# Maxwell-Zhao/RoboSimGS

Hardware: AMD Instinct MI355X
Metric: frames/sec + ms/frame (fwd, fwd+bwd) at 1M Gaussians 1920x1080 (higher is better)
Workload: dtype f32

## Files before the change

### robosimgs_amd/csrc/binning.hip

```cpp
#include "mgs_common.h"
#include "tile_rect.h"
#include "tile_order.h"

namespace mgs {
namespace {

constexpr int kBlock = 128;

__device__ __forceinline__ uint32_t wave_sum(uint32_t v) {
#pragma unroll
  for (int d = 32; d >= 1; d >>= 1) v += __shfl_xor(v, d);
  return v;
}

constexpr int kSum = 64;
__global__ __launch_bounds__(kBlock) void tile_count_kernel(
    int n, const float* __restrict__ means2d, const int32_t* __restrict__ radii,
    const int32_t* __restrict__ radii_y, const float* __restrict__ conics, const float* __restrict__ opacities,
    float tile_size, int tile_w, int tile_h, uint2* __restrict__ ginfo, uint32_t* __restrict__ sums) {
  int g = blockIdx.x * kBlock + threadIdx.x;
  int radius = g < n ? radii[g] : 0;
  uint2 info = make_uint2(kEmptyTileRect, 0u);
  if (radius > 0) {
    float2 m = reinterpret_cast<const float2*>(means2d)[g];
    TileRect r = tile_rect(m.x, m.y, radius, radii_y ? radii_y[g] : radius, tile_size, tile_w, tile_h);
    if (conics)
      r = tighten_rect(r, m.x, m.y, conics[3 * (size_t)g], conics[3 * (size_t)g + 1],
                       conics[3 * (size_t)g + 2], opacities[g], tile_size);
    info = pack_tile_rect(r);
  }
  if (g < n) ginfo[g] = info;
  const uint32_t c = wave_sum(info.y);
  const int first = blockIdx.x * kBlock + (int)(threadIdx.x & ~63u);
  if ((threadIdx.x & 63) == 0 && first < n) sums[first / kSum] = c;
}

constexpr int kScanThreads = 1024;
constexpr int kScanPerThread = 16;
template <int kScanThreads>
__device__ __forceinline__ void scan_blocksums_body(
    uint32_t nblk, uint32_t* __restrict__ blocksums, uint32_t capacity,
    uint32_t* __restrict__ n_isect, uint32_t* __restrict__ status) {
  __shared__ uint32_t ws[kScanThreads / 64];
  const unsigned lane = threadIdx.x & 63, wave = threadIdx.x >> 6;
  uint32_t running = 0;
  bool wrapped = false;
  for (uint32_t b0 = 0; b0 < nblk; b0 += kScanThreads * kScanPerThread) {
    const uint32_t b = b0 + threadIdx.x * kScanPerThread;
    uint32_t v[kScanPerThread], sum = 0;
    if (b + kScanPerThread <= nblk) {
      const uint4* src = reinterpret_cast<const uint4*>(blocksums + b);
      const uint4 q0 = src[0], q1 = src[1], q2 = src[2], q3 = src[3];
      v[0] = q0.x; v[1] = q0.y; v[2] = q0.z; v[3] = q0.w; v[4] = q1.x; v[5] = q1.y; v[6] = q1.z; v[7] = q1.w;
      v[8] = q2.x; v[9] = q2.y; v[10] = q2.z; v[11] = q2.w; v[12] = q3.x; v[13] = q3.y; v[14] = q3.z; v[15] = q3.w;
    } else {
#pragma unroll
      for (int j = 0; j < kScanPerThread; ++j) v[j] = b + j < nblk ? blocksums[b + j] : 0u;
    }
#pragma unroll
    for (int j = 0; j < kScanPerThread; ++j) sum += v[j];
    uint32_t incl = sum;
#pragma unroll
    for (int d = 1; d < 64; d <<= 1) {
      uint32_t t = __shfl_up(incl, d);
      if (lane >= (unsigned)d) incl += t;
    }
    if (lane == 63) ws[wave] = incl;
    __syncthreads();
    uint32_t off = 0, tot = 0;
    for (int w = 0; w < kScanThreads / 64; ++w) {
      if ((unsigned)w < wave) off += ws[w];
      tot += ws[w];
    }
    __syncthreads();
    uint32_t ex = running + off + incl - sum;
    uint32_t o[kScanPerThread];
#pragma unroll
    for (int j = 0; j < kScanPerThread; ++j) { o[j] = ex; ex += v[j]; }
    if (b + kScanPerThread <= nblk) {
      uint4* dst = reinterpret_cast<uint4*>(blocksums + b);
      dst[0] = make_uint4(o[0], o[1], o[2], o[3]);
      dst[1] = make_uint4(o[4], o[5], o[6], o[7]);
      dst[2] = make_uint4(o[8], o[9], o[10], o[11]);
      dst[3] = make_uint4(o[12], o[13], o[14], o[15]);
    } else {
#pragma unroll
      for (int j = 0; j < kScanPerThread; ++j)
        if (b + j < nblk) blocksums[b + j] = o[j];
    }
    wrapped |= running + tot < running;
    running += tot;
  }
  if (threadIdx.x == 0 && n_isect) {
    *n_isect = wrapped ? 0xffffffffu : running;
    *status = (wrapped || running > capacity) ? MGS_STATUS_ISECT_OVERFLOW : 0u;
  }
}
__global__ __launch_bounds__(kScanThreads) void scan_blocksums_kernel(
    uint32_t nblk, uint32_t* __restrict__ blocksums, uint32_t capacity,
    uint32_t* __restrict__ n_isect, uint32_t* __restrict__ status) {
  scan_blocksums_body<kScanThreads>(nblk, blocksums, capacity, n_isect, status);
}

__device__ __forceinline__ void store_splat_slots(float* __restrict__ splat_slots, int g, uint32_t slot_base, uint32_t rect) {
  if (splat_slots)
    *reinterpret_cast<uint2*>(splat_slots + 12 * (size_t)g + 10) = make_uint2(slot_base, rect & 0x3fffffffu);
}

__global__ __launch_bounds__(kBlock) void pair_info_kernel(
    int n, const uint2* __restrict__ ginfo, int tile_h, const uint32_t* __restrict__ blockbase,
    int4* __restrict__ pair_info, float* __restrict__ splat_slots) {
  __shared__ uint32_t ws[kBlock / 64];
  const unsigned lane = threadIdx.x & 63, wave = threadIdx.x >> 6;
  int g = blockIdx.x * kBlock + threadIdx.x;
  uint2 info = g < n ? ginfo[g] : make_uint2(1u << 20, 0u);
  uint32_t cnt = info.y;
  uint32_t incl = cnt;
#pragma unroll
  for (int d = 1; d < 64; d <<= 1) {
    uint32_t t = __shfl_up(incl, d);
    if (lane >= (unsigned)d) incl += t;
  }
  if (lane == 63) ws[wave] = incl;
  __syncthreads();
  uint32_t off = 0;
  for (int w = 0; w < kBlock / 64; ++w)
    if ((unsigned)w < wave) off += ws[w];
  if (g < n) {
    const uint32_t w = info.x >> 20;
    const uint32_t slot_base = blockbase[blockIdx.x * (kBlock / kSum)] + off + incl - cnt;
    pair_info[g] = cnt ? make_int4((int)slot_base, (int)(info.x & 1023u),
                                   (int)((info.x >> 10) & 1023u), (int)(w | ((cnt / w) << 16)))
                       : make_int4(0, 0, 0, 0);
    if (cnt) store_splat_slots(splat_slots, g, slot_base, info.x);
  }
}

__global__ __launch_bounds__(kBlock) void emit_kernel(
    int n, const uint2* __restrict__ ginfo, int tile_w, const uint32_t* __restrict__ blockbase,
    uint32_t capacity, uint32_t* __restrict__ tile_out, uint32_t* __restrict__ id_out,
    int32_t* __restrict__ tiles_per_gauss) {
  __shared__ uint32_t prefix[kBlock + 1];
  __shared__ uint32_t gid[kBlock];
  __shared__ uint32_t rpack[kBlock];
  __shared__ uint32_t ws[kBlock / 64];
  const unsigned lane = threadIdx.x & 63, wave = threadIdx.x >> 6;
  int r = blockIdx.x * kBlock + threadIdx.x;
  uint32_t cnt = 0, g = (uint32_t)r, pack = 1u << 20;
  if (r < n) {
    uint2 info = ginfo[r];
    pack = info.x;
    cnt = info.y;
    if (tiles_per_gauss) tiles_per_gauss[r] = (int32_t)cnt;
  }
  uint32_t incl = cnt;
#pragma unroll
  for (int d = 1; d < 64; d <<= 1) {
    uint32_t t = __shfl_up(incl, d);
    if (lane >= (unsigned)d) incl += t;
  }
  if (lane == 63) ws[wave] = incl;
  __syncthreads();
  uint32_t off = 0, total = 0;
  for (int w = 0; w < kBlock / 64; ++w) {
    if ((unsigned)w < wave) off += ws[w];
    total += ws[w];
  }
  prefix[threadIdx.x] = off + incl - cnt;
  if (threadIdx.x == 0) prefix[kBlock] = total;
  gid[threadIdx.x] = g;
  rpack[threadIdx.x] = pack;
  __syncthreads();
  const uint32_t base = blockbase[blockIdx.x * (kBlock / kSum)];
  for (uint32_t k0 = threadIdx.x * 4u; k0 < total; k0 += kBlock * 4u) {
    int lo = 0, hi = kBlock;
    while (hi - lo > 1) {
      int mid = (lo + hi) >> 1;
      if (prefix[mid] <= k0) lo = mid; else hi = mid;
    }
    uint32_t next = prefix[lo + 1];
    uint32_t tiles4[4], ids4[4];
#pragma unroll
    for (int i = 0; i < 4; ++i) {
      uint32_t k = k0 + i;
      while (k >= next && lo < kBlock - 1) next = prefix[++lo + 1];
      uint32_t local = k - prefix[lo];
      uint32_t p = rpack[lo];
      uint32_t w = p >> 20;
      uint32_t dy = local / w;
      uint32_t dx = local - dy * w;
      tiles4[i] = (((p >> 10) & 1023u) + dy) * (uint32_t)tile_w + (p & 1023u) + dx;
      ids4[i] = gid[lo];
    }
#pragma unroll
    for (int i = 0; i < 4; ++i) {
      uint32_t out = base + k0 + i;
      if (k0 + i < total && out < capacity) {
        tile_out[out] = tiles4[i];
        id_out[out] = ids4[i];
      }
    }
  }
}


constexpr int kDirectThreads = 512;
constexpr int kDealRun = 256;
static_assert(kDealRun % 64 == 0 && kDirectThreads % kDealRun == 0 && kDirectThreads >= kDealRun,
              "kDirectThreads must be a multiple of kDealRun, and the run a multiple of the wave");
constexpr int kDirectPerThread = 4;
constexpr int kDirectMaxBlocks = 1024;
constexpr int kDirectMaxTiles = 15000;
constexpr int kGroupShift = 2;
constexpr uint32_t kCoopRect = 24;
constexpr uint32_t kRunRect = 128;

template <class F>
__device__ __forceinline__ void for_each_tile(uint32_t pack, uint32_t cnt, uint32_t g, int tile_w, F f) {
  const bool big = cnt > kCoopRect;
  if (!big) {
    const uint32_t w = pack >> 20;
    uint32_t t = ((pack >> 10) & 1023u) * (uint32_t)tile_w + (pack & 1023u), dx = 0;
    for (uint32_t k = 0; k < cnt; ++k) {
      f(t + dx, g);
      if (++dx == w) { dx = 0; t += (uint32_t)tile_w; }
    }
  }
  unsigned long long m = ballot(big);
  const unsigned lane = lane_id();
  while (m) {
    const int src = __ffsll((long long)m) - 1;
    m &= m - 1;
    const uint32_t p = __shfl(pack, src), c = __shfl(cnt, src), gs = __shfl(g, src);
    const uint32_t w = p >> 20, x0 = p & 1023u, y0 = (p >> 10) & 1023u;
    for (uint32_t k = lane; k < c; k += 64) {
      const uint32_t dy = k / w, dx = k - dy * w;
      f((y0 + dy) * (uint32_t)tile_w + x0 + dx, gs);
    }
  }
}

template <class F>
__device__ __forceinline__ void for_each_tile_run(uint32_t pack, uint32_t cnt, uint32_t g, int tile_w, int shift, F f) {
  const bool big = cnt > kCoopRect;
  if (!big) {
    const uint32_t w = pack >> 20;
    uint32_t t = ((pack >> 10) & 1023u) * (uint32_t)tile_w + (pack & 1023u), dx = 0;
    for (uint32_t k = 0; k < cnt; ++k) {
      f(t + dx, 1u, g);
      if (++dx == w) { dx = 0; t += (uint32_t)tile_w; }
    }
  }
  unsigned long long m = ballot(big);
  const unsigned lane = lane_id();
  const uint32_t G = 1u << shift;
  while (m) {
    const int src = __ffsll((long long)m) - 1;
    m &= m - 1;
    const uint32_t p = __shfl(pack, src), c = __shfl(cnt, src), gs = __shfl(g, src);
    const uint32_t w = p >> 20, x0 = p & 1023u, y0 = (p >> 10) & 1023u, h = c / w;
    const uint32_t R = (w + G - 2u) / G + 1u;
    const int lr = R > 1u ? 32 - __clz((int)(R - 1u)) : 0;
    if (lr > 6 || c <= kRunRect) {
      for (uint32_t k = lane; k < c; k += 64) {
        const uint32_t dy = k / w, dx = k - dy * w;
        f((y0 + dy) * (uint32_t)tile_w + x0 + dx, 1u, gs);
      }
      continue;
    }
    const uint32_t rows_per_trip = 64u >> lr, r = lane >> lr, j = lane & ((1u << lr) - 1u);
    for (uint32_t dy0 = 0; dy0 < h; dy0 += rows_per_trip) {
      const uint32_t dy = dy0 + r;
      const uint32_t t0 = (y0 + dy) * (uint32_t)tile_w + x0, bin = (t0 >> shift) + j;
      const uint32_t lo = max(t0, bin << shift), hi = min(t0 + w, (bin + 1u) << shift);
      if (dy < h && lo < hi) f(lo, hi - lo, gs);
    }
  }
}

struct DealtIndex {
  int g0, g1, n, deal_nb;
  __device__ __forceinline__ int operator()(int base, int i) const {
    if (deal_nb > 0) {
      const int pass = (base - g0) / (kDirectThreads * kDirectPerThread);
      constexpr int R = kDealRun, kSub = kDirectThreads / R;
      const int sub = (int)threadIdx.x / R, within = (int)threadIdx.x % R;
      const long long g = (((long long)(pass * kDirectPerThread + i) * kSub + sub) * deal_nb + blockIdx.x) * R + within;
      return g < n ? (int)g : -1;
    }
    const int g = base + i * kDirectThreads + (int)threadIdx.x;
    return g < g1 ? g : -1;
  }
};

__global__ __launch_bounds__(kDirectThreads) void direct_hist_kernel(
    int n, int chunk, const uint2* __restrict__ ginfo, int tile_w, int n_tiles, int shift,
    uint32_t* __restrict__ table, int32_t* __restrict__ tiles_per_gauss, uint32_t* __restrict__ scan_sums, uint32_t n_sums,
    int deal_nb) {
  extern __shared__ uint32_t hist[];
  if (scan_sums && blockIdx.x == gridDim.x - 1) {
    scan_blocksums_body<kDirectThreads>(n_sums, scan_sums, 0u, nullptr, nullptr);
    return;
  }
  n_tiles = (n_tiles + (1 << shift) - 1) >> shift;
  for (int i = threadIdx.x; i < n_tiles; i += kDirectThreads) hist[i] = 0u;
  __syncthreads();
  const int g0 = blockIdx.x * chunk, g1 = min(n, g0 + chunk);
  const DealtIndex gi{g0, g1, n, deal_nb};
  const int g_end = deal_nb > 0 ? g0 + chunk : g1;
  for (int base = g0; base < g_end; base += kDirectThreads * kDirectPerThread) {
    uint2 info[kDirectPerThread];
#pragma unroll
    for (int i = 0; i < kDirectPerThread; ++i) {
      const int g = gi(base, i);
      info[i] = g >= 0 ? ginfo[g] : make_uint2(kEmptyTileRect, 0u);
    }
#pragma unroll
    for (int i = 0; i < kDirectPerThread; ++i) {
      const int g = gi(base, i);
      if (g >= 0 && tiles_per_gauss) tiles_per_gauss[g] = (int32_t)info[i].y;
      if (shift > 0)
        for_each_tile_run(info[i].x, info[i].y, (uint32_t)g, tile_w, shift, [&](uint32_t tile, uint32_t n_run, uint32_t) { atomicAdd(&hist[tile >> shift], n_run); });
      else
        for_each_tile(info[i].x, info[i].y, (uint32_t)g, tile_w, [&](uint32_t tile, uint32_t) { atomicAdd(&hist[tile >> shift], 1u); });
    }
  }
  __syncthreads();
  uint32_t* row = table + (size_t)blockIdx.x * n_tiles;
  for (int i = threadIdx.x; i < n_tiles; i += kDirectThreads) row[i] = hist[i];
}

constexpr int kColThreads = 256, kColBins = 16, kColGroups = kColThreads / kColBins, kColKeepTraining = 32;
template <int kColKeep>
__global__ __launch_bounds__(kColThreads) void direct_colscan_kernel(
    int nb, int n_tiles, uint32_t* __restrict__ table, uint32_t* __restrict__ tile_count) {
  __shared__ uint32_t part[kColGroups][kColBins];
  const int bl = threadIdx.x % kColBins, rg = threadIdx.x / kColBins;
  const int t = blockIdx.x * kColBins + bl;
  const int rpg = (nb + kColGroups - 1) / kColGroups;
  const int r0 = rg * rpg, r1 = min(nb, r0 + rpg);
  const bool ok = t < n_tiles;
  constexpr bool kCanKeep = kColKeep > 1;
  const bool keep = kCanKeep && rpg <= kColKeep;
  uint32_t kept[kColKeep];
  uint32_t sum = 0;
  if (kCanKeep && keep) {
#pragma unroll
    for (int j = 0; j < kColKeep; ++j) {
      if (j >= rpg) { kept[j] = 0u; continue; }
      kept[j] = (ok && r0 + j < r1) ? table[(size_t)(r0 + j) * n_tiles + t] : 0u;
    }
#pragma unroll
    for (int j = 0; j < kColKeep; ++j) sum += kept[j];
  } else {
    for (int r = r0; r < r1; r += 16) {
      uint32_t v[16];
#pragma unroll
      for (int j = 0; j < 16; ++j) v[j] = (ok && r + j < r1) ? table[(size_t)(r + j) * n_tiles + t] : 0u;
#pragma unroll
      for (int j = 0; j < 16; ++j) sum += v[j];
    }
  }
  part[rg][bl] = sum;
  __syncthreads();
  uint32_t off = 0, tot = 0;
#pragma unroll 16
  for (int g = 0; g < kColGroups; ++g) {
    const uint32_t s = part[g][bl];
    if (g < rg) off += s;
    tot += s;
  }
  if (kCanKeep && keep) {
#pragma unroll
    for (int j = 0; j < kColKeep; ++j) {
      if (j >= rpg) continue;
      if (ok && r0 + j < r1) {
        table[(size_t)(r0 + j) * n_tiles + t] = off;
        off += kept[j];
      }
    }
  } else {
    for (int r = r0; r < r1; r += 16) {
      uint32_t v[16];
#pragma unroll
      for (int j = 0; j < 16; ++j) v[j] = (ok && r + j < r1) ? table[(size_t)(r + j) * n_tiles + t] : 0u;
#pragma unroll
      for (int j = 0; j < 16; ++j)
        if (ok && r + j < r1) {
          table[(size_t)(r + j) * n_tiles + t] = off;
          off += v[j];
        }
    }
  }
  if (rg == 0 && ok) tile_count[t] = tot;
}

template <bool PAIRS>
__global__ __launch_bounds__(kDirectThreads) void direct_scatter_kernel(
    int n, int chunk, const uint2* __restrict__ ginfo, int tile_w, int n_tiles, int shift,
    const uint32_t* __restrict__ table, const uint32_t* __restrict__ tile_count, uint32_t capacity,
    uint32_t* __restrict__ flatten_ids, int32_t* __restrict__ tile_offsets,
    uint32_t* __restrict__ n_isect, uint32_t* __restrict__ status, int32_t* __restrict__ group_order,
    const uint32_t* __restrict__ scanned_sums, int4* __restrict__ pair_info, uint32_t* __restrict__ zero_word,
    float* __restrict__ splat_slots, int deal_nb) {
  extern __shared__ uint32_t cursor[];
  n_tiles = (n_tiles + (1 << shift) - 1) >> shift;
  if (group_order && blockIdx.x == gridDim.x - 1) {
    order_groups_by_total<kDirectThreads>(n_tiles, [&](int g) { return tile_count[g]; }, group_order);
    return;
  }
  const uint32_t local_mask = (1u << shift) - 1u;
  __shared__ unsigned long long wsum[kDirectThreads / 64];
  const unsigned lane = threadIdx.x & 63, wave = threadIdx.x >> 6;
  const int per = (n_tiles + kDirectThreads - 1) / kDirectThreads;
  const int t0 = (int)threadIdx.x * per;
  unsigned long long sum = 0;
  for (int k = 0; k < per; ++k)
    if (t0 + k < n_tiles) sum += tile_count[t0 + k];
  unsigned long long incl = sum;
#pragma unroll
  for (int d = 1; d < 64; d <<= 1) {
    const uint32_t lo = __shfl_up((uint32_t)incl, d), hi = __shfl_up((uint32_t)(incl >> 32), d);
    if (lane >= (unsigned)d) incl += ((unsigned long long)hi << 32) | lo;
  }
  if (lane == 63) wsum[wave] = incl;
  __syncthreads();
  unsigned long long off = 0, total = 0;
#pragma unroll
  for (int w = 0; w < kDirectThreads / 64; ++w) {
    if ((unsigned)w < wave) off += wsum[w];
    total += wsum[w];
  }
  unsigned long long ex = off + incl - sum;
  const uint32_t* row = table + (size_t)blockIdx.x * n_tiles;
  for (int k = 0; k < per; ++k) {
    const int t = t0 + k;
    if (t < n_tiles) {
      const uint32_t at = ex < capacity ? (uint32_t)ex : capacity;
      cursor[t] = ex < capacity ? at + row[t] : capacity;
      if (blockIdx.x == 0) tile_offsets[t] = (int32_t)at;
      ex += tile_count[t];
    }
  }
  if (blockIdx.x == 0 && threadIdx.x == 0) {
    tile_offsets[n_tiles] = (int32_t)(total < capacity ? (uint32_t)total : capacity);
    *n_isect = total > 0xffffffffull ? 0xffffffffu : (uint32_t)total;
    *status = total > capacity ? MGS_STATUS_ISECT_OVERFLOW : 0u;
    if (zero_word) reinterpret_cast<uint4*>(zero_word)[0] = reinterpret_cast<uint4*>(zero_word)[1] = make_uint4(0u, 0u, 0u, 0u);
  }
  __syncthreads();
  const int g0 = blockIdx.x * chunk, g1 = min(n, g0 + chunk);
  const DealtIndex gi{g0, g1, n, deal_nb};
  const int g_end = deal_nb > 0 ? g0 + chunk : g1;
  for (int base = g0; base < g_end; base += kDirectThreads * kDirectPerThread) {
    uint2 info[kDirectPerThread];
#pragma unroll
    for (int i = 0; i < kDirectPerThread; ++i) {
      const int g = gi(base, i);
      info[i] = g >= 0 ? ginfo[g] : make_uint2(kEmptyTileRect, 0u);
    }
    if (PAIRS) {
      uint32_t sbase[kDirectPerThread];
#pragma unroll
      for (int i = 0; i < kDirectPerThread; ++i) {
        const int g = gi(base, i);
        sbase[i] = g >= 0 ? scanned_sums[g / kSum] : 0u;
      }
#pragma unroll
      for (int i = 0; i < kDirectPerThread; ++i) {
        const int g = gi(base, i);
        const uint32_t cnt = info[i].y;
        uint32_t incl = cnt;
#pragma unroll
        for (int d = 1; d < 64; d <<= 1) {
          const uint32_t t = __shfl_up(incl, d);
          if (lane >= (unsigned)d) incl += t;
        }
        if (g >= 0) {
          const uint32_t w = info[i].x >> 20;
          pair_info[g] = cnt ? make_int4((int)(sbase[i] + incl - cnt), (int)(info[i].x & 1023u), (int)((info[i].x >> 10) & 1023u),
                                         (int)(w | ((cnt / w) << 16)))
                             : make_int4(0, 0, 0, 0);
          if (cnt) store_splat_slots(splat_slots, g, sbase[i] + incl - cnt, info[i].x);
        }
      }
    }
#pragma unroll
    for (int i = 0; i < kDirectPerThread; ++i) {
      const int g = gi(base, i);
      if (shift > 0)
        for_each_tile_run(info[i].x, info[i].y, (uint32_t)g, tile_w, shift, [&](uint32_t tile, uint32_t n_run, uint32_t gs) {
          const uint32_t p = atomicAdd(&cursor[tile >> shift], n_run);
          for (uint32_t k = 0; k < n_run; ++k)
            if (p + k < capacity) flatten_ids[p + k] = gs | (((tile + k) & local_mask) << (32 - shift));
        });
      else
      for_each_tile(info[i].x, info[i].y, (uint32_t)g, tile_w, [&](uint32_t tile, uint32_t gs) {
        const uint32_t p = atomicAdd(&cursor[tile >> shift], 1u);
        if (p < capacity) flatten_ids[p] = shift ? gs | ((tile & local_mask) << (32 - shift)) : gs;
      });
    }
  }
}

constexpr int kOffsetsPerThread = 8;
__global__ __launch_bounds__(kBlock) void tile_offsets_kernel(
    const uint32_t* __restrict__ n_ptr, uint32_t capacity, const uint32_t* __restrict__ tiles,
    int n_tiles, int32_t* __restrict__ offsets) {
  uint32_t n = min(*n_ptr, capacity);
  uint32_t t = blockIdx.x * kBlock + threadIdx.x;
  if (n == 0) {
    for (uint32_t k = t; k <= (uint32_t)n_tiles; k += gridDim.x * kBlock) offsets[k] = 0;
    return;
  }
  uint32_t i0 = t * kOffsetsPerThread;
  if (i0 >= n) return;
  uint32_t v[kOffsetsPerThread];
  if (i0 + kOffsetsPerThread <= n) {
    const uint4 a = *reinterpret_cast<const uint4*>(tiles + i0), b = *reinterpret_cast<const uint4*>(tiles + i0 + 4);
    v[0] = a.x; v[1] = a.y; v[2] = a.z; v[3] = a.w; v[4] = b.x; v[5] = b.y; v[6] = b.z; v[7] = b.w;
  } else {
#pragma unroll
    for (int j = 0; j < kOffsetsPerThread; ++j) v[j] = i0 + j < n ? tiles[i0 + j] : 0u;
  }
  int prev = i0 ? (int)tiles[i0 - 1] : -1;
#pragma unroll
  for (int j = 0; j < kOffsetsPerThread; ++j) {
    const uint32_t i = i0 + j;
    if (i < n) {
      const int cur = (int)v[j];
      for (int k = prev + 1; k <= cur; ++k) offsets[k] = (int32_t)i;
      prev = cur;
      if (i == n - 1)
        for (int k = cur + 1; k <= n_tiles; ++k) offsets[k] = (int32_t)n;
    }
  }
}

__global__ __launch_bounds__(kBlock) void isect_ids_kernel(
    const uint32_t* __restrict__ n_ptr, uint32_t capacity, const uint32_t* __restrict__ tiles,
    const int32_t* __restrict__ ids, const float* __restrict__ depths, int64_t cam_shifted,
    int64_t* __restrict__ isect_ids) {
  uint32_t n = min(*n_ptr, capacity);
  uint32_t i = blockIdx.x * kBlock + threadIdx.x;
  if (i >= n) return;
  int64_t hi = cam_shifted | (int64_t)tiles[i];
  isect_ids[i] = (hi << 32) | (int64_t)__float_as_uint(depths[ids[i]]);
}

__global__ __launch_bounds__(kBlock) void offset_encode_kernel(
    uint32_t n, const int64_t* __restrict__ isect_ids, int n_cams, int n_tiles, int tile_bits,
    int32_t* __restrict__ offsets) {
  uint32_t i = blockIdx.x * kBlock + threadIdx.x;
  int total = n_cams * n_tiles;
  if (n == 0) {
    for (uint32_t k = i; k < (uint32_t)total; k += gridDim.x * kBlock) offsets[k] = 0;
    return;
  }
  if (i >= n) return;
  auto flat = [&](int64_t key) {
    int64_t t = key >> 32;
    return (int)((t >> tile_bits) * n_tiles + (t & ((1ll << tile_bits) - 1)));
  };
  int cur = flat(isect_ids[i]);
  int prev = i ? flat(isect_ids[i - 1]) : -1;
  for (int k = prev + 1; k <= cur && k < total; ++k) offsets[k] = (int32_t)i;
  if (i == n - 1)
    for (int k = cur + 1; k < total; ++k) offsets[k] = (int32_t)n;
}

__global__ __launch_bounds__(1024) void tile_group_order_kernel(int n_tiles, const int32_t* __restrict__ tile_offsets,
                                                                int32_t* __restrict__ order) {
  order_groups_by_total<1024>((n_tiles + 3) / 4, [&](int g) {
    return (uint32_t)(tile_offsets[min(4 * g + 4, n_tiles)] - tile_offsets[4 * g]);
  }, order);
}

int bits_for(uint32_t count) {
  int b = 0;
  while (count > 1 && (1ull << b) < count) ++b;
  return b;
}

unsigned direct_chunk(unsigned n) {
  const unsigned per_block = max(div_up(n, kDirectMaxBlocks), (unsigned)(kDirectThreads * kDirectPerThread));
  return div_up(per_block, kDirectThreads) * kDirectThreads;
}
unsigned direct_blocks(unsigned n) { return div_up(n, direct_chunk(n)); }

struct Workspace {
  size_t total;
  size_t ginfo, blocksums, tile_alt, tile_priv, id_alt, radix, tsort, table, tile_count, group_offsets;
  Workspace(int n, uint32_t cap, int n_tiles) {
    Bump b(0);
    size_t nn = (size_t)(n > 0 ? n : 1), cc = cap ? cap : 1;
    ginfo = b.take(nn * 8);
    blocksums = b.take((size_t)div_up((unsigned)nn, kSum) * 4);
    tile_alt = b.take(cc * 4); id_alt = b.take(cc * 4);
    tile_priv = b.take(cc * 4);
    radix = b.take(radix_sort_temp_bytes((uint32_t)cc));
    tsort = b.take(tile_depth_sort_temp_bytes((uint32_t)cc, n_tiles));
    const size_t nt = (size_t)(n_tiles < kDirectMaxTiles ? n_tiles : kDirectMaxTiles);
    table = b.take((size_t)direct_blocks((unsigned)nn) * nt * 4);
    tile_count = b.take(nt * 4);
    group_offsets = b.take((nt + 1) * 4);
    total = b.total;
  }
};

}
}

namespace mgs {
size_t isect_tiles_workspace_bytes(int n, uint32_t capacity, int n_tiles) { return Workspace(n, capacity, n_tiles).total; }

int launch_tile_group_order(int n_tiles, const int32_t* tile_offsets, int32_t* order, hipStream_t stream) {
  hipLaunchKernelGGL(tile_group_order_kernel, dim3(1), dim3(1024), 0, stream, n_tiles, tile_offsets, order);
  return check_launch("tile_group_order");
}
}

using namespace mgs;

extern "C" int mgs_isect_tiles(int n, const float* means2d, const int32_t* radii, const int32_t* radii_y,
                               const float* depths, const float* conics, const float* opacities,
                               int tile_size, int tile_w, int tile_h,
                               int cam_id, int n_cams, uint32_t isect_capacity,
                               int32_t* tiles_per_gauss, uint32_t* n_isect, uint32_t* tile_ids,
                               int32_t* flatten_ids, int64_t* isect_ids, int32_t* tile_offsets,
                               int32_t* pair_info, int32_t* tile_group_order, uint32_t* status,
                               const uint32_t* seed_info,
                               uint32_t* seed_sums, float* splat_slots, void* workspace,
                               size_t* workspace_bytes, mgs_stream_t stream) {
  MGS_REQUIRE(n >= 0 && tile_size > 0 && tile_w > 0 && tile_h > 0, "isect_tiles: bad sizes");
  MGS_REQUIRE(tile_w <= 1023 && tile_h <= 1023, "isect_tiles: tile grid %dx%d exceeds 1023x1023", tile_w, tile_h);
  MGS_REQUIRE(workspace_bytes, "isect_tiles: workspace_bytes is null");
  MGS_REQUIRE(cam_id >= 0 && n_cams > cam_id, "isect_tiles: cam_id %d outside 0..%d", cam_id, n_cams);
  const Workspace ws(n, isect_capacity, tile_w * tile_h);
  if (!workspace) {
    *workspace_bytes = ws.total;
    return MGS_OK;
  }
  if (*workspace_bytes < ws.total)
    return set_error(MGS_ERR_WORKSPACE_TOO_SMALL, "isect_tiles: workspace %zu < %zu bytes",
                     *workspace_bytes, ws.total);
  MGS_REQUIRE(isect_capacity > 0, "isect_tiles: zero capacity");
  MGS_REQUIRE(seed_info || (conics == nullptr) == (opacities == nullptr),
              "isect_tiles: tight tile bounds need both conics and opacities");
  MGS_REQUIRE(n == 0 || (seed_info == nullptr) == (seed_sums == nullptr),
              "isect_tiles: seed_info and seed_sums come together (mgs_project_color_fwd writes both)");
  MGS_REQUIRE((n == 0 || ((seed_info || (means2d && radii)) && depths)) && n_isect && flatten_ids &&
                  tile_offsets && status, "isect_tiles: null pointer");
  MGS_REQUIRE(!seed_info || tile_size == MGS_TILE_SIZE, "isect_tiles: a seed is for tile_size %d, got %d", MGS_TILE_SIZE, tile_size);
  MGS_REQUIRE(!seed_sums || (reinterpret_cast<uintptr_t>(seed_sums) & 15u) == 0, "isect_tiles: seed_sums must be 16-byte aligned");
  MGS_REQUIRE(!splat_slots || pair_info, "isect_tiles: splat_slots are written with pair_info");
  MGS_REQUIRE(!splat_slots || (reinterpret_cast<uintptr_t>(splat_slots) & 15u) == 0, "isect_tiles: splat_slots must be 16-byte aligned");
  hipStream_t s = (hipStream_t)stream;
  char* w = static_cast<char*>(workspace);
  auto u32 = [&](size_t off) { return reinterpret_cast<uint32_t*>(w + off); };
  const bool want_tile_ids = tile_ids != nullptr;
  if (!tile_ids) tile_ids = u32(ws.tile_priv);
  const int n_tiles = tile_w * tile_h;
  const uint32_t cap = isect_capacity;
  const int gshift = (sort_opts() & 8) ? (sort_opts() >> 4) & 7 : kGroupShift;
  const bool direct = ((n_tiles + (1 << gshift) - 1) >> gshift) <= kDirectMaxTiles && !(sort_opts() & 4) &&
                      (gshift == 0 || (unsigned)n <= (1u << (32 - gshift)));
  int rc;
  bool order_done = false;

  if (n == 0) {
    (void)hipMemsetAsync(n_isect, 0, 4, s);
    (void)hipMemsetAsync(status, 0, 4, s);
  } else {
    const unsigned nblk = div_up(n, kBlock), nsum = div_up(n, kSum);
    const uint2* ginfo = reinterpret_cast<const uint2*>(seed_info);
    uint32_t* sums = seed_sums;
    if (!seed_info) {
      uint2* gi = reinterpret_cast<uint2*>(w + ws.ginfo);
      sums = u32(ws.blocksums);
      hipLaunchKernelGGL(tile_count_kernel, dim3(nblk), dim3(kBlock), 0, s, n, means2d, radii, radii_y, conics,
                         opacities, (float)tile_size, tile_w, tile_h, gi, sums);
      ginfo = gi;
    }
    if (direct) {
      const int chunk = (int)direct_chunk((unsigned)n);
      const unsigned nb = direct_blocks((unsigned)n);
      const int bins = (n_tiles + (1 << gshift) - 1) >> gshift;
      const size_t lds = (size_t)bins * sizeof(uint32_t);
      const int deal_nb = (int)nb;
      hipLaunchKernelGGL(direct_hist_kernel, dim3(nb + (pair_info ? 1 : 0)), dim3(kDirectThreads), lds, s, n, chunk, ginfo, tile_w,
                         n_tiles, gshift, u32(ws.table), tiles_per_gauss, pair_info ? sums : nullptr, nsum, deal_nb);
      if (pair_info)
        hipLaunchKernelGGL(direct_colscan_kernel<kColKeepTraining>, dim3(div_up((unsigned)bins, (unsigned)kColBins)), dim3(kColThreads), 0, s,
                           (int)nb, bins, u32(ws.table), u32(ws.tile_count));
      else
        hipLaunchKernelGGL(direct_colscan_kernel<1>, dim3(div_up((unsigned)bins, (unsigned)kColBins)), dim3(kColThreads), 0, s,
                           (int)nb, bins, u32(ws.table), u32(ws.tile_count));
      const bool order_in_scatter = tile_group_order && gshift == 2;
      order_done = order_in_scatter;
      with_bool(pair_info != nullptr, [&](auto training) {
        hipLaunchKernelGGL(direct_scatter_kernel<decltype(training)::value>, dim3(nb + (order_in_scatter ? 1 : 0)),
                           dim3(kDirectThreads), lds, s, n, chunk, ginfo, tile_w, n_tiles, gshift, u32(ws.table),
                           u32(ws.tile_count), cap, gshift ? u32(ws.id_alt) : reinterpret_cast<uint32_t*>(flatten_ids),
                           gshift ? reinterpret_cast<int32_t*>(w + ws.group_offsets) : tile_offsets, n_isect, status,
                           order_in_scatter ? tile_group_order : nullptr, sums, reinterpret_cast<int4*>(pair_info),
                           tile_depth_sort_long_list(w + ws.tsort, cap), pair_info ? splat_slots : nullptr, deal_nb);
      });
    } else {
      hipLaunchKernelGGL(scan_blocksums_kernel, dim3(1), dim3(kScanThreads), 0, s, nsum, sums, cap,
                         n_isect, status);
      const int tile_bits = bits_for((uint32_t)n_tiles);
      const int passes = (tile_bits + 7) / 8;
      uint32_t* user_t = tile_ids;
      uint32_t* user_i = reinterpret_cast<uint32_t*>(flatten_ids);
      uint32_t *a_t = user_t, *a_i = user_i, *b_t = u32(ws.tile_alt), *b_i = u32(ws.id_alt);
      if (passes & 1) { a_t = u32(ws.tile_alt); a_i = u32(ws.id_alt); b_t = user_t; b_i = user_i; }
      hipLaunchKernelGGL(emit_kernel, dim3(nblk), dim3(kBlock), 0, s, n, ginfo, tile_w, sums, cap, a_t,
                         a_i, tiles_per_gauss);
      if (pair_info)
        hipLaunchKernelGGL(pair_info_kernel, dim3(nblk), dim3(kBlock), 0, s, n, ginfo, tile_h, sums,
                           reinterpret_cast<int4*>(pair_info), splat_slots);
      rc = radix_sort_pairs(n_isect, cap, tile_bits, a_t, a_i, b_t, b_i, w + ws.radix, s);
      if (rc) return rc;
    }
  }
  if (!direct || n == 0)
    hipLaunchKernelGGL(tile_offsets_kernel, dim3(div_up(cap, kBlock * kOffsetsPerThread)), dim3(kBlock), 0,
                       s, n_isect, cap, tile_ids, n_tiles, tile_offsets);
  if (n > 0) {
    const bool grouped = direct && gshift > 0;
    rc = tile_depth_sort(n_tiles, tile_offsets, depths, cap, reinterpret_cast<uint32_t*>(flatten_ids),
                         direct && (want_tile_ids || isect_ids) ? tile_ids : nullptr, w + ws.tsort, s,
                          u32(ws.tile_alt), u32(ws.id_alt),
                         grouped ? u32(ws.id_alt) : nullptr,
                         grouped ? reinterpret_cast<const int32_t*>(w + ws.group_offsets) : nullptr, gshift, direct);
    if (rc) return rc;
  }
  if (tile_group_order && !order_done) {
    rc = launch_tile_group_order(n_tiles, tile_offsets, tile_group_order, s);
    if (rc) return rc;
  }
  const unsigned gblk = div_up(cap, kBlock);
  if (isect_ids) {
    const int tile_bits_key = bits_for((uint32_t)n_tiles + 1);
    hipLaunchKernelGGL(isect_ids_kernel, dim3(gblk), dim3(kBlock), 0, s, n_isect, cap, tile_ids,
                       flatten_ids, depths, (int64_t)cam_id << tile_bits_key, isect_ids);
  }
  return check_launch("isect_tiles");
}

extern "C" int mgs_isect_offset_encode(uint32_t n_isect, const int64_t* isect_ids, int n_cams,
                                       int tile_w, int tile_h, int32_t* offsets,
                                       mgs_stream_t stream) {
  MGS_REQUIRE(n_cams > 0 && tile_w > 0 && tile_h > 0, "isect_offset_encode: bad sizes");
  MGS_REQUIRE(offsets && (isect_ids || n_isect == 0), "isect_offset_encode: null pointer");
  const int n_tiles = tile_w * tile_h;
  const int tile_bits = bits_for((uint32_t)n_tiles + 1);
  unsigned gblk = n_isect ? div_up(n_isect, kBlock) : div_up((unsigned)(n_cams * n_tiles), kBlock);
  hipLaunchKernelGGL(offset_encode_kernel, dim3(gblk), dim3(kBlock), 0, (hipStream_t)stream,
                     n_isect, isect_ids, n_cams, n_tiles, tile_bits, offsets);
  return check_launch("isect_offset_encode");
}
```

### robosimgs_amd/csrc/build.py

```python
from __future__ import annotations

import hashlib
import os
import shutil
import subprocess
import sys
from concurrent.futures import ThreadPoolExecutor

HERE = os.path.dirname(os.path.abspath(__file__))
SOURCES = ["api.hip", "projection.hip", "sort.hip", "binning.hip", "tile_sort.hip", "raster_fwd.hip",
           "raster_bwd.hip", "backward.hip", "composite.hip", "points.hip", "loss.hip", "transform.hip", "frame.hip"]
HEADERS = ["mgs_common.h", "mgs_math.h", "raster_common.h", "sh_staging.h", "tile_rect.h", "tile_order.h",
           "../../include/mgs.h"]
LIB = os.path.join(HERE, "libmgs.so")
DEBUG_LIB = os.path.join(HERE, "libmgs_debug.so")
HOOK_SOURCES = ["raster_fwd.hip", "sort.hip"]
OBJ_DIR = os.path.join(HERE, "build")
FLAGS = ["--offload-arch=gfx950", "-O3", "-std=c++17", "-fPIC", "-munsafe-fp-atomics",
         "-fno-slp-vectorize", "-Wall", "-Wno-unused-function"] + os.environ.get("MGS_EXTRA_FLAGS", "").split()


PER_SOURCE_FLAGS = {
    "raster_bwd.hip": os.environ.get("MGS_RASTER_BWD_FLAGS", "").split(),
    "raster_fwd.hip": os.environ.get("MGS_RASTER_FWD_FLAGS", "").split(),
    "tile_sort.hip": os.environ.get("MGS_TILE_SORT_FLAGS", "").split(),
    "binning.hip": os.environ.get("MGS_BINNING_FLAGS", "").split(),
}


def _hipcc() -> str:
    for c in (os.environ.get("HIPCC"), shutil.which("hipcc"), "/opt/rocm/bin/hipcc"):
        if c and os.path.exists(c):
            return c
    raise RuntimeError("hipcc not found; libmgs.so cannot be built")


def _stamp() -> str:
    h = hashlib.sha256((" ".join(FLAGS) + repr(sorted(PER_SOURCE_FLAGS.items()))).encode())
    for f in SOURCES + HEADERS:
        p = os.path.join(HERE, f)
        if os.path.exists(p):
            with open(p, "rb") as fh:
                h.update(fh.read())
    return h.hexdigest()


def _code_only(text: str) -> str:
    out, i, n = [], 0, len(text)
    while i < n:
        c = text[i]
        if c in "\"'":
            j = i + 1
            while j < n and text[j] != c:
                j += 2 if text[j] == "\\" else 1
            out.append(text[i:j + 1])
            i = j + 1
        elif text.startswith("//", i):
            j = text.find("\n", i)
            i = n if j < 0 else j
        elif text.startswith("/*", i):
            j = text.find("*/", i + 2)
            i = n if j < 0 else j + 2
            out.append(" ")
        else:
            out.append(c)
            i += 1
    return " ".join("".join(out).split())


def current_stamp() -> str:
    h = hashlib.sha256((" ".join(FLAGS) + repr(sorted(PER_SOURCE_FLAGS.items()))).encode())
    for f in SOURCES + HEADERS:
        p = os.path.join(HERE, f)
        if os.path.exists(p):
            with open(p, "r", encoding="utf-8", errors="replace") as fh:
                h.update(_code_only(fh.read()).encode())
    return h.hexdigest()


def build(force: bool = False, verbose: bool = False) -> str:
    stamp_file = os.path.join(OBJ_DIR, "stamp")
    stamp = _stamp()
    if (not force and os.path.exists(LIB) and os.path.exists(DEBUG_LIB) and os.path.exists(stamp_file)
            and open(stamp_file).read() == stamp):
        return LIB
    os.makedirs(OBJ_DIR, exist_ok=True)
    hipcc = _hipcc()
    srcs = [s for s in SOURCES if os.path.exists(os.path.join(HERE, s))]

    def compile_one(job) -> str:
        src, hooks = job
        obj = os.path.join(OBJ_DIR, src.replace(".hip", ".dbg.o" if hooks else ".o"))
        cmd = [hipcc, *FLAGS, *PER_SOURCE_FLAGS.get(src, []), *(["-DMGS_DEBUG_HOOKS"] if hooks else []), "-c",
               os.path.join(HERE, src), "-o", obj]
        if verbose:
            print(" ".join(cmd), flush=True)
        r = subprocess.run(cmd, capture_output=True, text=True)
        if r.returncode != 0:
            raise RuntimeError(f"hipcc failed on {src}:\n{r.stderr}")
        if verbose and r.stderr.strip():
            print(r.stderr, file=sys.stderr)
        return obj

    jobs = [(s_, False) for s_ in srcs] + [(s_, True) for s_ in srcs if s_ in HOOK_SOURCES]
    with ThreadPoolExecutor(max_workers=4) as ex:
        objs = dict(zip(jobs, ex.map(compile_one, jobs)))
    for lib, hooks in ((LIB, False), (DEBUG_LIB, True)):
        use = [objs[(s_, hooks and s_ in HOOK_SOURCES)] for s_ in srcs]
        cmd = [hipcc, "--offload-arch=gfx950", "-shared", "-fPIC", *use, "-o", lib]
        r = subprocess.run(cmd, capture_output=True, text=True)
        if r.returncode != 0:
            raise RuntimeError(f"link failed:\n{r.stderr}")
    with open(stamp_file, "w") as f:
        f.write(stamp)
    return LIB


if __name__ == "__main__":
    print(build(force="--force" in sys.argv, verbose=True))
```

Before: 4410.

## Replace column-scan kernel with atomic per-tile range reservation in histogram

Each histogram block now reserves its slice of every tile's range by atomically adding its local count to a global per-tile counter, and writes the returned base into the table. This removes the separate column-scan kernel launch and its reads and writes of the whole block-by-tile table. The counters are zeroed inside tile_count_kernel, or by a small new kernel when seed info is provided. Per-block offsets within a tile are no longer in block order, so the order of Gaussians within a tile becomes nondeterministic, which may affect depth ordering unless it is sorted later. The old column scan is kept only in the debug build.

```diff
diff --git a/robosimgs_amd/csrc/binning.hip b/robosimgs_amd/csrc/binning.hip
--- a/robosimgs_amd/csrc/binning.hip
+++ b/robosimgs_amd/csrc/binning.hip
@@ -17,8 +17,10 @@
 __global__ __launch_bounds__(kBlock) void tile_count_kernel(
     int n, const float* __restrict__ means2d, const int32_t* __restrict__ radii,
     const int32_t* __restrict__ radii_y, const float* __restrict__ conics, const float* __restrict__ opacities,
-    float tile_size, int tile_w, int tile_h, uint2* __restrict__ ginfo, uint32_t* __restrict__ sums) {
+    float tile_size, int tile_w, int tile_h, uint2* __restrict__ ginfo, uint32_t* __restrict__ sums,
+    uint32_t* __restrict__ zero_counters, int n_counters) {
   int g = blockIdx.x * kBlock + threadIdx.x;
+  for (int i = g; i < n_counters; i += gridDim.x * kBlock) zero_counters[i] = 0u;
   int radius = g < n ? radii[g] : 0;
   uint2 info = make_uint2(kEmptyTileRect, 0u);
   if (radius > 0) {
@@ -33,6 +35,11 @@
   const uint32_t c = wave_sum(info.y);
   const int first = blockIdx.x * kBlock + (int)(threadIdx.x & ~63u);
   if ((threadIdx.x & 63) == 0 && first < n) sums[first / kSum] = c;
+}
+
+__global__ __launch_bounds__(256) void zero_counters_kernel(uint32_t* __restrict__ counters, int n) {
+  const int i = blockIdx.x * 256 + threadIdx.x;
+  if (i < n) counters[i] = 0u;
 }
 
 constexpr int kScanThreads = 1024;
@@ -296,7 +303,7 @@
 __global__ __launch_bounds__(kDirectThreads) void direct_hist_kernel(
     int n, int chunk, const uint2* __restrict__ ginfo, int tile_w, int n_tiles, int shift,
     uint32_t* __restrict__ table, int32_t* __restrict__ tiles_per_gauss, uint32_t* __restrict__ scan_sums, uint32_t n_sums,
-    int deal_nb) {
+    int deal_nb, uint32_t* __restrict__ tile_count) {
   extern __shared__ uint32_t hist[];
   if (scan_sums && blockIdx.x == gridDim.x - 1) {
     scan_blocksums_body<kDirectThreads>(n_sums, scan_sums, 0u, nullptr, nullptr);
@@ -327,11 +334,20 @@
   }
   __syncthreads();
   uint32_t* row = table + (size_t)blockIdx.x * n_tiles;
-  for (int i = threadIdx.x; i < n_tiles; i += kDirectThreads) row[i] = hist[i];
-}
-
-constexpr int kColThreads = 256, kColBins = 16, kColGroups = kColThreads / kColBins, kColKeepTraining = 32;
-template <int kColKeep>
+#ifdef MGS_DEBUG_HOOKS
+  if (!tile_count) {
+    for (int i = threadIdx.x; i < n_tiles; i += kDirectThreads) row[i] = hist[i];
+    return;
+  }
+#endif
+  for (int i = threadIdx.x; i < n_tiles; i += kDirectThreads) {
+    const uint32_t c = hist[i];
+    row[i] = c ? atomicAdd(&tile_count[i], c) : 0u;
+  }
+}
+
+#ifdef MGS_DEBUG_HOOKS
+constexpr int kColThreads = 256, kColBins = 16, kColGroups = kColThreads / kColBins;
 __global__ __launch_bounds__(kColThreads) void direct_colscan_kernel(
     int nb, int n_tiles, uint32_t* __restrict__ table, uint32_t* __restrict__ tile_count) {
   __shared__ uint32_t part[kColGroups][kColBins];
@@ -340,60 +356,24 @@
   const int rpg = (nb + kColGroups - 1) / kColGroups;
   const int r0 = rg * rpg, r1 = min(nb, r0 + rpg);
   const bool ok = t < n_tiles;
-  constexpr bool kCanKeep = kColKeep > 1;
-  const bool keep = kCanKeep && rpg <= kColKeep;
-  uint32_t kept[kColKeep];
   uint32_t sum = 0;
-  if (kCanKeep && keep) {
-#pragma unroll
-    for (int j = 0; j < kColKeep; ++j) {
-      if (j >= rpg) { kept[j] = 0u; continue; }
-      kept[j] = (ok && r0 + j < r1) ? table[(size_t)(r0 + j) * n_tiles + t] : 0u;
-    }
-#pragma unroll
-    for (int j = 0; j < kColKeep; ++j) sum += kept[j];
-  } else {
-    for (int r = r0; r < r1; r += 16) {
-      uint32_t v[16];
-#pragma unroll
-      for (int j = 0; j < 16; ++j) v[j] = (ok && r + j < r1) ? table[(size_t)(r + j) * n_tiles + t] : 0u;
-#pragma unroll
-      for (int j = 0; j < 16; ++j) sum += v[j];
-    }
-  }
+  for (int r = r0; r < r1; ++r) sum += ok ? table[(size_t)r * n_tiles + t] : 0u;
   part[rg][bl] = sum;
   __syncthreads();
   uint32_t off = 0, tot = 0;
-#pragma unroll 16
   for (int g = 0; g < kColGroups; ++g) {
     const uint32_t s = part[g][bl];
     if (g < rg) off += s;
     tot += s;
   }
-  if (kCanKeep && keep) {
-#pragma unroll
-    for (int j = 0; j < kColKeep; ++j) {
-      if (j >= rpg) continue;
-      if (ok && r0 + j < r1) {
-        table[(size_t)(r0 + j) * n_tiles + t] = off;
-        off += kept[j];
-      }
-    }
-  } else {
-    for (int r = r0; r < r1; r += 16) {
-      uint32_t v[16];
-#pragma unroll
-      for (int j = 0; j < 16; ++j) v[j] = (ok && r + j < r1) ? table[(size_t)(r + j) * n_tiles + t] : 0u;
-#pragma unroll
-      for (int j = 0; j < 16; ++j)
-        if (ok && r + j < r1) {
-          table[(size_t)(r + j) * n_tiles + t] = off;
-          off += v[j];
-        }
-    }
+  for (int r = r0; r < r1 && ok; ++r) {
+    const uint32_t v = table[(size_t)r * n_tiles + t];
+    table[(size_t)r * n_tiles + t] = off;
+    off += v;
   }
   if (rg == 0 && ok) tile_count[t] = tot;
 }
+#endif
 
 template <bool PAIRS>
 __global__ __launch_bounds__(kDirectThreads) void direct_scatter_kernel(
@@ -675,27 +655,34 @@
     const unsigned nblk = div_up(n, kBlock), nsum = div_up(n, kSum);
     const uint2* ginfo = reinterpret_cast<const uint2*>(seed_info);
     uint32_t* sums = seed_sums;
+    const int bins = (n_tiles + (1 << gshift) - 1) >> gshift;
+#ifdef MGS_DEBUG_HOOKS
+    const bool reserve = direct && !(sort_opts() & 128);
+#else
+    const bool reserve = direct;
+#endif
     if (!seed_info) {
       uint2* gi = reinterpret_cast<uint2*>(w + ws.ginfo);
       sums = u32(ws.blocksums);
       hipLaunchKernelGGL(tile_count_kernel, dim3(nblk), dim3(kBlock), 0, s, n, means2d, radii, radii_y, conics,
-                         opacities, (float)tile_size, tile_w, tile_h, gi, sums);
+                         opacities, (float)tile_size, tile_w, tile_h, gi, sums, u32(ws.tile_count), reserve ? bins : 0);
       ginfo = gi;
+    } else if (reserve) {
+      hipLaunchKernelGGL(zero_counters_kernel, dim3(div_up((unsigned)bins, 256u)), dim3(256), 0, s, u32(ws.tile_count), bins);
     }
     if (direct) {
       const int chunk = (int)direct_chunk((unsigned)n);
       const unsigned nb = direct_blocks((unsigned)n);
-      const int bins = (n_tiles + (1 << gshift) - 1) >> gshift;
       const size_t lds = (size_t)bins * sizeof(uint32_t);
       const int deal_nb = (int)nb;
       hipLaunchKernelGGL(direct_hist_kernel, dim3(nb + (pair_info ? 1 : 0)), dim3(kDirectThreads), lds, s, n, chunk, ginfo, tile_w,
-                         n_tiles, gshift, u32(ws.table), tiles_per_gauss, pair_info ? sums : nullptr, nsum, deal_nb);
-      if (pair_info)
-        hipLaunchKernelGGL(direct_colscan_kernel<kColKeepTraining>, dim3(div_up((unsigned)bins, (unsigned)kColBins)), dim3(kColThreads), 0, s,
+                         n_tiles, gshift, u32(ws.table), tiles_per_gauss, pair_info ? sums : nullptr, nsum, deal_nb,
+                         reserve ? u32(ws.tile_count) : nullptr);
+#ifdef MGS_DEBUG_HOOKS
+      if (!reserve)
+        hipLaunchKernelGGL(direct_colscan_kernel, dim3(div_up((unsigned)bins, (unsigned)kColBins)), dim3(kColThreads), 0, s,
                            (int)nb, bins, u32(ws.table), u32(ws.tile_count));
-      else
-        hipLaunchKernelGGL(direct_colscan_kernel<1>, dim3(div_up((unsigned)bins, (unsigned)kColBins)), dim3(kColThreads), 0, s,
-                           (int)nb, bins, u32(ws.table), u32(ws.tile_count));
+#endif
       const bool order_in_scatter = tile_group_order && gshift == 2;
       order_done = order_in_scatter;
       with_bool(pair_info != nullptr, [&](auto training) {
diff --git a/robosimgs_amd/csrc/build.py b/robosimgs_amd/csrc/build.py
--- a/robosimgs_amd/csrc/build.py
+++ b/robosimgs_amd/csrc/build.py
@@ -14,7 +14,7 @@
            "../../include/mgs.h"]
 LIB = os.path.join(HERE, "libmgs.so")
 DEBUG_LIB = os.path.join(HERE, "libmgs_debug.so")
-HOOK_SOURCES = ["raster_fwd.hip", "sort.hip"]
+HOOK_SOURCES = ["raster_fwd.hip", "sort.hip", "binning.hip"]
 OBJ_DIR = os.path.join(HERE, "build")
 FLAGS = ["--offload-arch=gfx950", "-O3", "-std=c++17", "-fPIC", "-munsafe-fp-atomics",
          "-fno-slp-vectorize", "-Wall", "-Wno-unused-function"] + os.environ.get("MGS_EXTRA_FLAGS", "").split()
```

Result: no change. 4465, median of 3 (+1.3%).
